# zju3dv/Mirror-NeRF

Measured on AMD Instinct MI355X. Metric: rendered rays/sec (primary+reflected), higher is better.
Workload: dtype f32 carried as hi/lo f16 pairs (f16 MFMA, f32 accumulate; max |diff| to the fp32 chain 3e-6)

## Files before the change

include/mnrf.h:

```cpp
#ifndef MNRF_H
#define MNRF_H

#include <stdint.h>

#ifdef __cplusplus
extern "C" {
#endif

#define MNRF_OK 0
#define MNRF_ERR_ARG (-1)
#define MNRF_ERR_LAUNCH (-2)
#define MNRF_ERR_UNSUPPORTED (-3)

#define MNRF_N_PARAMS 32

#define MNRF_SIGMA_ONLY 1u
#define MNRF_GRAD_NORMAL 2u
#define MNRF_SPLIT_F16 4u

#define MNRF_TCNN_GRAD_F16 16u
#define MNRF_TCNN_GRAD_FIXED 512u
#define MNRF_TCNN_F16 256u
#define MNRF_TCNN_TABLE_F16 1024u
#define MNRF_TCNN_VALU 8u
// ... 114 lines not shown
                         const float* normal, const float* save_invj, const uint64_t* save_mask,
                         float* workspace, float* const* d_params, float* d_xyz, unsigned flags , void* stream);

int mnrf_tcnn_encode(const float* table, const int64_t* offsets17_host, double log2_per_level_scale, int base_resolution,
                     float bound, int64_t B, const float* xyz, int64_t xyz_stride, const float* rays, const float* z_vals,
                     int spr, float* planes, void* stream);

int mnrf_tcnn_encode_flags(const float* table, const int64_t* offsets17_host, double log2_per_level_scale, int base_resolution,
                           float bound, int64_t B, const float* xyz, int64_t xyz_stride, const float* rays, const float* z_vals,
                           int spr, float* planes, unsigned flags, void* stream);
int mnrf_tcnn_table_half(const float* table, int64_t entries, void* table_half, void* stream);

int mnrf_bench_gather(const void* table, int64_t table_bytes, int bytes_per_gather, int64_t n_threads, int iters, float* out,
                      void* stream);

int mnrf_fused_samples_per_ray(void);
int mnrf_field_composite_fused(float* packed, int64_t n_rays, const float* rays, const float* z_vals,
                               const float* dir_emb, int64_t dir_stride, int white_back,
                               float* weights, float* opacity, float* rgb_map, float* depth, float* mirror_mask,
                               float* surf_normal, float* x_surface, void* stream);

#define MNRF_TRAIN_PLANES 256u
#define MNRF_PLANES_Y_HALF 0x100000u
int64_t mnrf_train_planes_bytes(int64_t B);
int64_t mnrf_train_dy_planes_bytes(int64_t B);

int mnrf_field_backward_planes(float* packed, int64_t B, const float* xyz, int64_t xyz_stride,
                               const float* rays, const float* z_vals, int spr,
                               const float* g_sigma, const float* g_rgb, const float* g_pred_normal,
                               const float* g_is_mirror, const float* rgb, const float* pred_normal,
                               const float* is_mirror, const uint64_t* save_mask, const float* save_inv,
                               void* dy_planes, uint32_t* seedmax, float* d_xyz, float* d_dir, const float* keep_mirror,
                               unsigned flags ,
// ... 194 lines not shown
```

mirror_nerf_amd/_lib.py:

```python
import ctypes
import os
import subprocess

import torch

_HERE = os.path.dirname(os.path.abspath(__file__))
LIB_PATH = os.environ.get("MNRF_LIB", os.path.join(_HERE, "libmnrf_hip.so"))
CSRC = os.path.join(_HERE, "csrc")

_c_f = ctypes.c_void_p
_c_i = ctypes.c_void_p
_i64 = ctypes.c_int64
_int = ctypes.c_int
_u32 = ctypes.c_uint
_flt = ctypes.c_float
_str = ctypes.c_void_p

MNRF_SIGMA_ONLY = 1
MNRF_GRAD_NORMAL = 2
MNRF_SPLIT_F16 = 4
MNRF_TCNN_VALU = 8
MNRF_TCNN_F16 = 256
MNRF_TCNN_GRAD_FIXED = 512
MNRF_TCNN_TABLE_F16 = 1024
MNRF_CUT_NORMAL_HEAD = 32
MNRF_CUT_MIRROR_HEAD = 64
MNRF_DW_ACCUMULATE = 128
MNRF_TRAIN_PLANES = 256
MNRF_PLANES_Y_HALF = 0x100000
MNRF_TCNN_GRAD_F16 = 16
MNRF_DETACH_W_MASK = 1
MNRF_DETACH_W_NORMAL = 2
N_PARAMS = 32

SIGNATURES = {
# ... 166 lines not shown
```

mirror_nerf_amd/csrc/mnrf_composite.inc:

```
struct CompMaps {
    float* weights;
    float* opacity; float* rgb_map; float* depth; float* mirror_mask;
    float* surf_normal; float* surf_normal_grad; float* normal_dif; float* x_surface;
    const float* rays;
    int white_back;
};

template <class Src>
__device__ __forceinline__ void composite_ray(const Src& src, int S, int lane, long long ray, const CompMaps& A) {
    float carry = 1.f;
    float a_op = 0.f, a_d = 0.f, a_m = 0.f, a_nd = 0.f;
    float a_c[3] = {0.f, 0.f, 0.f}, a_n[3] = {0.f, 0.f, 0.f}, a_g[3] = {0.f, 0.f, 0.f};
    for (int base = 0; base < S; base += 64) {
        const int s = base + lane;
        const bool in = s < S;
        float alpha = 0.f, zv = 0.f;
        if (in) {
            zv = src.z(s);
            const float delta = s + 1 < S ? src.z(s + 1) - zv : 1e10f;
            float sv = src.sigma(s);
            if (src.has_noise()) sv = sv + src.noise(s);
            alpha = 1.f - expf(-delta * fmaxf(sv, 0.f));
        }
        const float t = in ? (1.f - alpha) + 1e-10f : 1.f;
// ... 18 lines not shown
#pragma unroll
                for (int k = 0; k < 3; ++k) { pn[k] = src.pn(s, k); a_n[k] += pn[k] * w; }
            }
            if (src.has_gn()) {
#pragma unroll
                for (int k = 0; k < 3; ++k) { gn[k] = src.gn(s, k); a_g[k] += gn[k] * w; }
            }
            if (src.has_pn() && src.has_gn()) {
                const float d0 = gn[0] - pn[0], d1 = gn[1] - pn[1], d2 = gn[2] - pn[2];
                a_nd += w * (d0 * d0 + d1 * d1 + d2 * d2);
            }
        }
    }
    a_op = wave_sum(a_op);
    a_d = wave_sum(a_d);
    a_m = wave_sum(a_m);
    a_nd = wave_sum(a_nd);
#pragma unroll
    for (int k = 0; k < 3; ++k) { a_c[k] = wave_sum(a_c[k]); a_n[k] = wave_sum(a_n[k]); a_g[k] = wave_sum(a_g[k]); }
    if (lane == 0) {
        if (A.opacity) A.opacity[ray] = a_op;
        if (A.rgb_map) {
#pragma unroll
            for (int k = 0; k < 3; ++k) A.rgb_map[ray * 3 + k] = A.white_back ? a_c[k] + (1.f - a_op) : a_c[k];
        }
        if (A.depth) A.depth[ray] = a_d;
        if (A.mirror_mask) A.mirror_mask[ray] = a_m;
        if (A.surf_normal) { for (int k = 0; k < 3; ++k) A.surf_normal[ray * 3 + k] = a_n[k]; }
        if (A.surf_normal_grad) { for (int k = 0; k < 3; ++k) A.surf_normal_grad[ray * 3 + k] = a_g[k]; }
        if (A.normal_dif) A.normal_dif[ray] = a_nd;
        if (A.x_surface) {
            const float* r = A.rays + ray * 8;
            for (int k = 0; k < 3; ++k) A.x_surface[ray * 3 + k] = r[k] + r[3 + k] * a_d;
        }
// ... 3 lines not shown
```

mirror_nerf_amd/csrc/mnrf_field.hip:

```cpp
#include <hip/hip_runtime.h>
#include <stdint.h>
#include <stdlib.h>

#include "mnrf_layout.h"
#include "mnrf_field_args.h"

namespace mnrf {

extern __shared__ __attribute__((aligned(16))) char smem[];

namespace s2 {
constexpr int S = 2;
constexpr int MIN_WAVES_PER_SIMD = 1;
constexpr int CHUNK_TILES = 16;
#include "mnrf_field_impl.inc"
#include "mnrf_field_bwd.inc"
}
namespace s1 {
constexpr int S = 1;
constexpr int MIN_WAVES_PER_SIMD = 2;
constexpr int CHUNK_TILES = 16;
#include "mnrf_field_impl.inc"
}

// ... 144 lines not shown
    if (!xyz && B % spr != 0) return mnrf_fail(MNRF_ERR_ARG, "mnrf_field_forward: B not a multiple of spr");
    if (!sigma_only && !dir_emb) return mnrf_fail(MNRF_ERR_ARG, "mnrf_field_forward: dir_emb required unless SIGMA_ONLY");
    if (grad && !normal) return mnrf_fail(MNRF_ERR_ARG, "mnrf_field_forward: GRAD_NORMAL needs the normal output");
    FieldArgs A{packed, flags, (long long)B, xyz, (long long)xyz_stride, rays, z_vals, spr, dir_emb,
                (long long)dir_stride, sigma, rgb, pred_normal, is_mirror, normal, geo_feat};
    const int rc = (flags & MNRF_SPLIT_F16) ? launch_split(A, sigma_only, grad, (hipStream_t)stream)
                 : grad ? s1::launch(A, sigma_only, grad, (hipStream_t)stream)
                        : s2::launch(A, sigma_only, grad, (hipStream_t)stream);
    if (rc != 0) return mnrf_fail(MNRF_ERR_ARG, "mnrf_field_forward: too many samples for one launch");
    return mnrf_check_launch("mnrf_field_forward");
}

extern "C" int mnrf_fused_samples_per_ray(void) { return split48_ray_samples(); }

extern "C" int mnrf_field_composite_fused(float* packed, int64_t n_rays, const float* rays, const float* z_vals,
                                          const float* dir_emb, int64_t dir_stride, int white_back,
                                          float* weights, float* opacity, float* rgb_map, float* depth, float* mirror_mask,
                                          float* surf_normal, float* x_surface, void* stream) {
    if (!packed || !rays || !z_vals || !dir_emb) return mnrf_fail(MNRF_ERR_ARG, "mnrf_field_composite_fused: null pointer");
    if (n_rays < 0) return mnrf_fail(MNRF_ERR_ARG, "mnrf_field_composite_fused: negative ray count");
    if (n_rays == 0) return MNRF_OK;
    if (!split48_enabled())
        return mnrf_fail(MNRF_ERR_UNSUPPORTED, "mnrf_field_composite_fused: needs the 48-samples-per-wave tuning (MNRF_SPLIT48 != 0)");
    const int spr = split48_ray_samples();
    FieldArgs A{packed, MNRF_SPLIT_F16, (long long)n_rays * spr, nullptr, 3, rays, z_vals, spr, dir_emb, (long long)dir_stride,
                nullptr, nullptr, nullptr, nullptr, nullptr, nullptr};
    A.fuse = 1;
    A.white_back = white_back;
    A.f_weights = weights; A.f_opacity = opacity; A.f_rgb_map = rgb_map; A.f_depth = depth; A.f_mirror_mask = mirror_mask;
    A.f_surf_normal = surf_normal; A.f_x_surface = x_surface;
    if (launch_split48(A, false, (hipStream_t)stream) != 0)
        return mnrf_fail(MNRF_ERR_ARG, "mnrf_field_composite_fused: too many samples for one launch");
    return mnrf_check_launch("mnrf_field_composite_fused");
}

static inline int64_t train_tiles(int64_t B) { return (B + s2::WG_SAMPLES - 1) / s2::WG_SAMPLES; }

extern "C" int64_t mnrf_train_save_floats(int64_t B) { return (int64_t)SAVE_FLOATS * B; }
extern "C" int64_t mnrf_train_mask_words(int64_t B) { return train_tiles(B) * N_MASKS * s2::S * s2::WG_THREADS; }
extern "C" int64_t mnrf_train_workspace_floats(int64_t B) { return (int64_t)DY_FLOATS * B + dw_workspace_floats(B); }

static int field_forward_train_impl(float* packed, int64_t B, const float* xyz, int64_t xyz_stride,
                                    const float* rays, const float* z_vals, int spr, const float* dir_emb,
// ... 246 lines not shown
```

mirror_nerf_amd/csrc/mnrf_field_split.hip:

```cpp
#include <hip/hip_runtime.h>
#include <stdint.h>
#include <type_traits>
#include <stdlib.h>

#include "mnrf_layout.h"
#include "mnrf_field_args.h"

namespace mnrf {

extern __shared__ __attribute__((aligned(16))) char smem[];

namespace h2 {
constexpr int S = 2;
constexpr int MIN_WAVES_PER_SIMD = 1;
constexpr int CHUNK_PAIRS = 8;
constexpr int RING_SLOTS = 4;
#include "mnrf_field_split.inc"
}
namespace h2x {
constexpr int S = 2;
constexpr int MIN_WAVES_PER_SIMD = 1;
constexpr int CHUNK_PAIRS = 16;
constexpr int RING_SLOTS = 3;
#include "mnrf_field_split.inc"
// ... 108 lines not shown
        } else if (b >= BIAS_DIR && b < BIAS_DIR + 128) {
            const float* wd = I.wdir[blockIdx.y] + (b - BIAS_DIR) * (W + ENC_DIR);
            double a = 0.0;
            for (int k = 0; k < W; ++k) a = fma((double)wd[k], (double)bias[BIAS_FIN + k], a);
            v = (float)(a + (double)bias[b]);
        }
        packed[OFF_FOLD_BIAS + b] = v;
        return;
    }
    const int pair = (int)(q >> 6);
    const int lane = (int)(q & 63);
    const int row = lane & 15;
    typedef _Float16 h8v __attribute__((ext_vector_type(8)));
    h8v hi, lo;
    for (int j = 0; j < 8; ++j) hi[j] = lo[j] = (_Float16)0.f;
    const int sp = pair < 968 ? pair : (pair < 1036 ? pair + (1036 - 968) : (pair >= 1100 && pair < 1112 ? pair + (1296 - 1100) : -1));
    if (sp >= 0) {
        const char* src = (const char*)(packed + OFF_SPLIT_FWD) + (long long)sp * PAIR_BYTES + lane * 16;
        hi = *(const h8v*)src;
        lo = *(const h8v*)(src + PAIR_BYTES / 2);
    }
    const bool fold_nrm = pair >= 960 && pair < 968 && row >= 1 && row <= 3;
    const bool fold_dir = pair >= 1036 && pair < 1100;
    if (fold_nrm || fold_dir) {
        const int T = fold_nrm ? pair - 960 : (pair - 1036) / 8;
        const int c0 = 32 * T + 4 * (lane >> 4);
        const float* a = fold_nrm ? I.wn2[blockIdx.y] + (row - 1) * 128 : I.wdir[blockIdx.y] + (16 * ((pair - 1036) % 8) + row) * (W + ENC_DIR);
        const float* bm = fold_nrm ? I.wn1[blockIdx.y] : I.wfin[blockIdx.y];
        const int K = fold_nrm ? 128 : W;
        double acc[8];
        for (int j = 0; j < 8; ++j) acc[j] = 0.0;
        for (int k = 0; k < K; ++k) {
            const double ak = (double)a[k];
            const float* bk = bm + (long long)k * W + c0;
#pragma unroll
            for (int c = 0; c < 4; ++c) {
                acc[c] = fma(ak, (double)bk[c], acc[c]);
                acc[4 + c] = fma(ak, (double)bk[16 + c], acc[4 + c]);
            }
        }
        bool bad = false;
#pragma unroll
// ... 28 lines not shown
```

mirror_nerf_amd/csrc/mnrf_field_split.inc:

```
constexpr int CHUNK_BYTES = CHUNK_PAIRS * PAIR_BYTES;
constexpr int WAVES = 4;
constexpr int WG_THREADS = 64 * WAVES;
constexpr int WG_SAMPLES = WAVES * S * 16;
constexpr int PIECES = CHUNK_BYTES / TILE_BYTES / WAVES;
constexpr int U = 2;
constexpr int PF = S == 3 ? 2 : 4;
constexpr int NBUF = PF + U;
typedef unsigned u32x4 __attribute__((ext_vector_type(4)));
typedef unsigned u32x2 __attribute__((ext_vector_type(2)));
typedef _Float16 h2v __attribute__((ext_vector_type(2)));
struct StoreCtx {
    __amdgpu_buffer_rsrc_t rsrc;
    __amdgpu_buffer_rsrc_t rsrc_lo;
    char* base;
    int lane;
    int soff;
    h2v fac[S];
};
__device__ __forceinline__ __amdgpu_buffer_rsrc_t plane_rsrc(char* sample_block) {
    return __builtin_amdgcn_make_buffer_rsrc(sample_block, 0, 0x7fffffff, 0x00020000);
}
static_assert(CHUNK_PAIRS / U == PIECES, "one LDS-DMA piece per wave per unit");
constexpr int LDS_RING = RING_SLOTS * CHUNK_BYTES;
constexpr int LDS_BIAS = LDS_RING;
// ... 21 lines not shown
struct CompLdsSrc {
    const float* f;
    bool pn_on, mir_on;
    __device__ __forceinline__ bool has_noise() const { return false; }
    __device__ __forceinline__ bool has_rgb() const { return true; }
    __device__ __forceinline__ bool has_mirror() const { return mir_on; }
    __device__ __forceinline__ bool has_pn() const { return pn_on; }
    __device__ __forceinline__ bool has_gn() const { return false; }
    __device__ __forceinline__ float z(int s) const { return f[8 * WG_SAMPLES + s]; }
    __device__ __forceinline__ float sigma(int s) const { return f[s]; }
    __device__ __forceinline__ float noise(int) const { return 0.f; }
    __device__ __forceinline__ float rgb(int s, int k) const { return f[(1 + k) * WG_SAMPLES + s]; }
    __device__ __forceinline__ float mirror(int s) const { return f[7 * WG_SAMPLES + s]; }
    __device__ __forceinline__ float pn(int s, int k) const { return f[(4 + k) * WG_SAMPLES + s]; }
    __device__ __forceinline__ float gn(int, int) const { return 0.f; }
};

__device__ __forceinline__ unsigned long long enc_out_of_range(const float (&x)[S][3]) {
    bool big = false;
#pragma unroll
    for (int s = 0; s < S; ++s) big |= !(fabsf(x[s][0]) < ENC_RANGE_LIMIT && fabsf(x[s][1]) < ENC_RANGE_LIMIT && fabsf(x[s][2]) < ENC_RANGE_LIMIT);
    return __builtin_amdgcn_ballot_w64(big);
}

template <int N>
__device__ __forceinline__ void split_b(const float (&x)[S][N], u32x4 (&hi)[S][N / 8], u32x4 (&lo)[S][N / 8],
                                        unsigned long long& sat, float limit = F16_MAX) {
    float tmax = 0.f;
#pragma unroll
    for (int s = 0; s < S; ++s)
// ... 337 lines not shown
            sat_track<ACT == 1>(tmax, v[2], v[3]);
            hi[s][nb >> 1][2 * (nb & 1)] = h0;
            hi[s][nb >> 1][2 * (nb & 1) + 1] = h1;
            lo[s][nb >> 1][2 * (nb & 1)] = l0;
            lo[s][nb >> 1][2 * (nb & 1) + 1] = l1;
        }
        if (WANT_MASK) ((uint64_t*)(smem + LDS_MASK))[(layer * S + s) * WG_THREADS + tid] = m;
    }
    sat_flush(sat, tmax);
}

__device__ __forceinline__ float sigmoidf_(float x) { return 1.f / (1.f + expf(-x)); }



template <bool SIGMA_ONLY, bool GRAD, bool PLANES = false, bool FUSE = false>
__global__ __launch_bounds__(WG_THREADS, MIN_WAVES_PER_SIMD) void field_split_kernel(FieldArgs A) {
    static_assert(!PLANES || (GRAD && !SIGMA_ONLY && S == 2), "operand planes: the training forward (32 samples per wave)");
    static_assert(!FUSE || (S == 3 && !SIGMA_ONLY && !GRAD), "ray-fused compositing: the 192-sample fine pass");
    constexpr bool FOLD = !SIGMA_ONLY && !GRAD;
    float* const fz = (float*)(smem + LDS_FUSE);
    constexpr bool PERSIST = S == 3;
    if constexpr (PLANES) {
        if (A.n_live) {
            long long bl = (long long)*A.n_live * A.spr;
            bl = bl < 0 ? 0 : bl;
            if (bl < A.B) A.B = bl;
        }
        if ((long long)blockIdx.x * WG_SAMPLES >= A.B) return;
    }
    const bool queued = PERSIST && A.tile_queue != nullptr;
    const int wave = __builtin_amdgcn_readfirstlane(threadIdx.x >> 6);
    int tile = blockIdx.x;
    int round = 0;
// ... 268 lines not shown
    };
    {
        f32x4 acc[S][1];
        init_bias<1>(acc, BIAS_SIG, gq());
        gemm_part<8, 1, 960, HP>(acc, hh, hl, st, wave, lane16);
        if (FUSE) {
            if (gq() == 0) {
#pragma unroll
                for (int s = 0; s < S; ++s) fz[wave * (S * 16) + s * 16 + m15()] = acc[s][0][0];
            }
        } else if (A.sigma && g == 0) {
#pragma unroll
            for (int s = 0; s < S; ++s)
                if (sval(s)) out_store(A.sigma + sidx(s), acc[s][0][0]);
        }
        if constexpr (FOLD) put_normal(acc, std::integral_constant<int, 1>{});
    }

    if (!SIGMA_ONLY) {
        if constexpr (!FOLD) {
            u32x4 nh[S][4], nl[S][4];
            {
                f32x4 acc[S][8];
                init_bias<8>(acc, BIAS_NRM1, gq());
                gemm_part<8, 8, 968, HP, ST0>(acc, hh, hl, st, wave, lane16, at_h(7, 0));
                if (keep) save_acc<8, 0>(A.save_x + (long long)SEC_HN * A.B, 128, 0, acc, idx, valid, g, unused_bits);
                acc_to_b<8, 0, false>(nh, nl, acc, 0, tid, st.sat);
                if constexpr (S == 2) { if (pl) store_planes<4, 4>(sc, SEC_HN / 16, nh, nl); }
            }
            f32x4 acc[S][1];
            init_bias<1>(acc, BIAS_NRM2, gq());
            gemm_part<4, 1, 1032>(acc, nh, nl, st, wave, lane16);
            put_normal(acc, std::integral_constant<int, 0>{});
        }
        {
            u32x4 mh[S][4], ml[S][4];
            {
                f32x4 acc[S][8];
                init_bias<8>(acc, BIAS_MIR1, gq());
                gemm_part<8, 8, FOLD ? 968 : 1036, HP, ST4>(acc, hh, hl, st, wave, lane16, at_h(7, 4));
                if (keep) {
                    uint64_t bits[S];
                    save_acc<8, 2>(A.save_x + (long long)SEC_HM * A.B, 128, 0, acc, idx, valid, g, bits);
#pragma unroll
                    for (int s = 0; s < S; ++s) gmask[(9 * S + s) * WG_THREADS + tid] = bits[s];
                } else if (GRAD && pl) {
                    store_sign_mask<8>(acc, gmask + (9 * S) * WG_THREADS + tid);
                }
                acc_to_b<8, 2, false>(mh, ml, acc, 0, tid, st.sat);
                if constexpr (S == 2) { if (pl) store_planes<4, 4>(sc, SEC_HM / 16, mh, ml); }
            }
            f32x4 acc[S][1];
            init_bias<1>(acc, BIAS_MIR2, gq());
            gemm_part<4, 1, FOLD ? 1032 : 1100>(acc, mh, ml, st, wave, lane16);
            if (FUSE) {
                if (gq() == 0) {
#pragma unroll
                    for (int s = 0; s < S; ++s) fz[7 * WG_SAMPLES + wave * (S * 16) + s * 16 + m15()] = sigmoidf_(acc[s][0][0]);
                }
            } else if (A.is_mirror && g == 0) {
#pragma unroll
                for (int s = 0; s < S; ++s)
                    if (sval(s)) out_store(A.is_mirror + sidx(s), sigmoidf_(acc[s][0][0]));
            }
        }
        const auto view_operands = [&](u32x4 (&vh)[S][1], u32x4 (&vl)[S][1]) {
            float de[S][8];
            const int gv = gq();
            const int spr = opaque_spr();
#pragma unroll
            for (int s = 0; s < S; ++s) {
                const float* dp = A.dir_emb + (long long)(sidx(s) / spr) * A.dir_stride;
#pragma unroll
                for (int t = 0; t < 8; ++t) {
                    const int e = 16 * (t >> 2) + 4 * gv + (t & 3);
                    de[s][t] = e < ENC_DIR ? dp[e] : 0.f;
                }
            }
            if (keep) save_bform<8>(A.save_x + (long long)SEC_DIRE * A.B, 32, de, idx, valid, g);
            split_b<8>(de, vh, vl, st.sat);
            if constexpr (S == 2) { if (pl) store_planes<1, 1>(sc, SEC_DIRE / 16, vh, vl); }
        };
        {
            u32x4 dh[S][4], dl[S][4];
            if constexpr (FOLD) {
                u32x4 vh[S][1], vl[S][1];
                view_operands(vh, vl);
                f32x4 acc[S][8];
                init_bias<8>(acc, BIAS_DIR, gq());
                gemm_part<8, 8, 1036, HP>(acc, hh, hl, st, wave, lane16);
                gemm_part<1, 8, 1100>(acc, vh, vl, st, wave, lane16);
                acc_to_b<8, 1, false>(dh, dl, acc, 0, tid, st.sat);
            } else {
                u32x4 fh[S][8], fl[S][8];
                {
                    f32x4 acc[S][16];
                    init_bias<16>(acc, BIAS_FIN, gq());
                    gemm_part<8, 16, 1104, HP>(acc, hh, hl, st, wave, lane16);
                    if (keep) save_acc<16, 0>(A.save_x + (long long)SEC_FIN * A.B, 256, 0, acc, idx, valid, g, unused_bits);
                    acc_to_b<16, 0, false>(fh, fl, acc, 0, tid, st.sat);
                    if constexpr (S == 2) { if (pl) store_planes<8, 8>(sc, SEC_FIN / 16, fh, fl); }
                }
                u32x4 vh[S][1], vl[S][1];
                view_operands(vh, vl);
                f32x4 acc[S][8];
                init_bias<8>(acc, BIAS_DIR, gq());
                gemm_part<8, 8, 1232>(acc, fh, fl, st, wave, lane16);
                gemm_part<1, 8, 1296>(acc, vh, vl, st, wave, lane16);
                if (keep) {
                    uint64_t bits[S];
                    save_acc<8, 1>(A.save_x + (long long)SEC_HD * A.B, 128, 0, acc, idx, valid, g, bits);
#pragma unroll
                    for (int s = 0; s < S; ++s) gmask[(8 * S + s) * WG_THREADS + tid] = bits[s];
                } else if (GRAD && pl) {
                    store_sign_mask<8>(acc, gmask + (8 * S) * WG_THREADS + tid);
                }
                acc_to_b<8, 1, false>(dh, dl, acc, 0, tid, st.sat);
                if constexpr (S == 2) { if (pl) store_planes<4, 4>(sc, SEC_HD / 16, dh, dl); }
            }
            f32x4 acc[S][1];
            init_bias<1>(acc, BIAS_RGB, gq());
            gemm_part<4, 1, FOLD ? 1108 : 1304>(acc, dh, dl, st, wave, lane16);
            if (FUSE) {
                if (gq() == 0) {
#pragma unroll
                    for (int s = 0; s < S; ++s) {
                        const int q = wave * (S * 16) + s * 16 + (int)m15();
                        fz[1 * WG_SAMPLES + q] = sigmoidf_(acc[s][0][0]);
                        fz[2 * WG_SAMPLES + q] = sigmoidf_(acc[s][0][1]);
                        fz[3 * WG_SAMPLES + q] = sigmoidf_(acc[s][0][2]);
                    }
                }
            } else if (A.rgb && g == 0) {
#pragma unroll
                for (int s = 0; s < S; ++s)
                    if (sval(s)) {
                        float* o = A.rgb + (long long)sidx(s) * 3;
                        out_store(o, sigmoidf_(acc[s][0][0]));
                        out_store(o + 1, sigmoidf_(acc[s][0][1]));
                        out_store(o + 2, sigmoidf_(acc[s][0][2]));
                    }
            }
        }
    }

    if (GRAD) {
        open_stream<false>(st, A.packed + OFF_SPLIT_BWD, wave, lane);
        prime_stream(st, lane16);
        float gr[S][64];
        {
            const f32x4* ws = (const f32x4*)(smem + LDS_BIAS) + (BIAS_WSIG >> 2);
#pragma unroll
            for (int nb = 0; nb < 16; ++nb) {
                const f32x4 v = ws[nb * 4 + g];
#pragma unroll
                for (int s = 0; s < S; ++s)
#pragma unroll
                    for (int r = 0; r < 4; ++r) gr[s][4 * nb + r] = v[r];
// ... 70 lines not shown
                const float n0 = -d0, n1 = -d1, n2 = -d2;
                const float sq = n0 * n0 + n1 * n1 + n2 * n2;
                const float inv = 1.f / sqrtf(fmaxf(sq, 1.1920928955078125e-07f));
                float* o = A.normal + (long long)idx[s] * 3;
                o[0] = n0 * inv; o[1] = n1 * inv; o[2] = n2 * inv;
                if (A.save_invj) A.save_invj[idx[s]] = sq > 1.1920928955078125e-07f ? inv : -inv;
            }
        }
    }
    sat_all |= st.sat;
    enc_all |= enc_range;
    if (FUSE) {
        __syncthreads();
        if (wave == 0) {
            const long long ray = tile;
            const CompLdsSrc src{fz, A.f_surf_normal != nullptr, A.f_mirror_mask != nullptr};
            const CompMaps out{A.f_weights ? A.f_weights + ray * WG_SAMPLES : nullptr, A.f_opacity, A.f_rgb_map, A.f_depth, A.f_mirror_mask,
                               A.f_surf_normal, nullptr, nullptr, A.f_x_surface, A.rays, A.white_back};
            int cl;
            asm volatile("v_mbcnt_lo_u32_b32 %0, -1, 0\n\tv_mbcnt_hi_u32_b32 %0, -1, %0" : "=v"(cl));
            composite_ray(src, WG_SAMPLES, cl, ray, out);
        }
    }
    if (!queued) break;
    close_stream();
    __syncthreads();
    tile = __builtin_amdgcn_readfirstlane(((volatile int*)(smem + LDS_TILEQ))[round & 1]);
    ++round;
    if (tile >= A.n_tiles) break;
    }
    guard_report(A.packed, sat_all, enc_all, MNRF_GUARD_IN_FORWARD);
    close_stream();
    int last_lane;
    asm volatile("v_mbcnt_lo_u32_b32 %0, -1, 0\n\tv_mbcnt_hi_u32_b32 %0, -1, %0" : "=v"(last_lane));
    if (queued && wave == 0 && last_lane == 0) {
        if (atomicAdd(A.tile_queue + 1, 1) == (int)gridDim.x - 1) {
            atomicExch(A.tile_queue, 0);
            atomicExch(A.tile_queue + 1, 0);
        }
    }
}

inline int launch(const FieldArgs& A, bool sigma_only, bool grad, hipStream_t s) {
    const long long blocks64 = (A.B + WG_SAMPLES - 1) / WG_SAMPLES;
    if (blocks64 > 0x7fffffff || A.B > 0x7fffffffLL) return -1;
    dim3 grid((unsigned)blocks64);
    const dim3 block(WG_THREADS);
    if (S == 3 && A.tile_queue) {
        if (A.n_tiles != (int)blocks64 || A.resident < 1 || A.resident > A.n_tiles) return -1;
        grid = dim3((unsigned)A.resident);
    }
    if (sigma_only && !grad) hipLaunchKernelGGL((field_split_kernel<true, false>), grid, block, LDS_BYTES, s, A);
    else if (!sigma_only && !grad && S == 3 && A.fuse)
        hipLaunchKernelGGL((field_split_kernel<false, false, false, S == 3>), grid, block, LDS_BYTES_FUSE, s, A);
    else if (!sigma_only && !grad) hipLaunchKernelGGL((field_split_kernel<false, false>), grid, block, LDS_BYTES, s, A);
#ifndef MNRF_SPLIT_NO_GRAD
    else if (sigma_only && grad) hipLaunchKernelGGL((field_split_kernel<true, true>), grid, block, LDS_BYTES_GRAD, s, A);
    else if (S == 2 && A.save_planes) hipLaunchKernelGGL((field_split_kernel<false, true, S == 2>), grid, block, LDS_BYTES_GRAD, s, A);
    else hipLaunchKernelGGL((field_split_kernel<false, true>), grid, block, LDS_BYTES_GRAD, s, A);
#else
    else return -1;
#endif
    return 0;
}
```

mirror_nerf_amd/csrc/mnrf_field_split3.hip:

```cpp
#include <hip/hip_runtime.h>
#include <stdint.h>
#include <type_traits>
#include <stdlib.h>

#include "mnrf_layout.h"
#include "mnrf_field_args.h"

namespace mnrf {

extern __shared__ __attribute__((aligned(16))) char smem[];

namespace h3 {
constexpr int S = 3;
constexpr int MIN_WAVES_PER_SIMD = 1;
constexpr int CHUNK_PAIRS = 8;
constexpr int RING_SLOTS = 4;
#define MNRF_SPLIT_NO_GRAD
#include "mnrf_field_split.inc"
#undef MNRF_SPLIT_NO_GRAD
}

bool split48_enabled() {
    static const bool v = [] { const char* e = getenv("MNRF_SPLIT48"); return !(e && atoi(e) == 0); }();
    return v;
// ... 20 lines not shown
    A.resident = resident;
    return true;
}

int launch_split48(const FieldArgs& A0, bool sigma_only, hipStream_t s) {
    FieldArgs A = A0;
    A.tile_queue = nullptr;
    if (tile_queue_slot(A)) {
        if (hipMemsetAsync(A.tile_queue, 0, 2 * sizeof(int), s) != hipSuccess) A.tile_queue = nullptr;
    }
    static const bool once = [] {
        (void)hipFuncSetAttribute((const void*)h3::field_split_kernel<true, false>, hipFuncAttributeMaxDynamicSharedMemorySize, h3::LDS_BYTES);
        (void)hipFuncSetAttribute((const void*)h3::field_split_kernel<false, false>, hipFuncAttributeMaxDynamicSharedMemorySize, h3::LDS_BYTES);
        (void)hipFuncSetAttribute((const void*)h3::field_split_kernel<false, false, false, true>, hipFuncAttributeMaxDynamicSharedMemorySize,
                                   h3::LDS_BYTES_FUSE);
        return true;
    }();
    (void)once;
    return h3::launch(A, sigma_only, false, s);
}

int split48_ray_samples() { return h3::WG_SAMPLES; }

}
```

mirror_nerf_amd/csrc/mnrf_layout.h:

```cpp
#pragma once
#include <stdint.h>

namespace mnrf {

constexpr int W = 256;
constexpr int ENC_XYZ = 63;
constexpr int ENC_DIR = 27;
constexpr int NFREQ_XYZ = 10;
constexpr int NFREQ_DIR = 4;

constexpr int TILE_FLOATS = 256;
constexpr int TILE_BYTES = 1024;
constexpr int PAD_TILES = 16;

enum PartKind : int {
    KIND_H = 0,
    KIND_ENC = 1,
    KIND_DIR = 2,
};

__host__ __device__ inline int enc_col(int t, int g) {
    const int P = 8 * g + (t >> 1);
    const int s = t & 1;
    if (P < 30) return 3 + 6 * (P / 3) + 3 * s + (P % 3);
// ... 42 lines not shown
constexpr int64_t PACKED_F32_FLOATS = OFF_HBWD + (int64_t)HBWD_TILES * TILE_FLOATS;

constexpr int PAIR_BYTES = 2048;
constexpr int SPLIT_END_PAD = 16;
__host__ __device__ constexpr int padded_pairs(int n) { return (n + SPLIT_END_PAD - 1) / SPLIT_END_PAD * SPLIT_END_PAD; }
constexpr int SPLIT_FWD_USED_SIGMA = 960 + 8;
constexpr int SPLIT_FWD_USED = SPLIT_FWD_USED_SIGMA + 64 + 4 + 64 + 4 + 128 + 64 + 8 + 4;
constexpr int SPLIT_FWD_PAIRS = padded_pairs(SPLIT_FWD_USED);
constexpr int SPLIT_BWD_PAIRS = 3 * 128 + 32 + 128 + 3 * 128 + 32;
constexpr int SPLIT_HBWD_PAIRS = padded_pairs(8 + 64 + 8 + 128 + 8 + 64 + 8 + 64);
constexpr int64_t OFF_SPLIT_FWD = PACKED_F32_FLOATS;
constexpr int64_t OFF_SPLIT_BWD = OFF_SPLIT_FWD + (int64_t)SPLIT_FWD_PAIRS * (PAIR_BYTES / 4);
constexpr int64_t OFF_SPLIT_HBWD = OFF_SPLIT_BWD + (int64_t)SPLIT_BWD_PAIRS * (PAIR_BYTES / 4);
constexpr int64_t SPLIT_TAIL_FLOATS = 2 * 16 * (PAIR_BYTES / 4);
constexpr int FOLD_REGION_PAIRS = 1328;
constexpr int SPLIT_FOLD_USED = 960 + 8 + 64 + 4 + 64 + 8 + 4;
constexpr int SPLIT_FOLD_PAIRS = padded_pairs(SPLIT_FOLD_USED);
constexpr int64_t OFF_FOLD_FWD = OFF_SPLIT_HBWD + (int64_t)SPLIT_HBWD_PAIRS * (PAIR_BYTES / 4);
constexpr int64_t OFF_FOLD_BIAS = OFF_FOLD_FWD + (int64_t)SPLIT_FOLD_PAIRS * (PAIR_BYTES / 4) + SPLIT_TAIL_FLOATS;
constexpr int64_t PACKED_FLOATS = OFF_FOLD_FWD + (int64_t)FOLD_REGION_PAIRS * (PAIR_BYTES / 4) + SPLIT_TAIL_FLOATS;
constexpr int TQ_PAIRS = 8;
constexpr int64_t OFF_TILE_QUEUE = PACKED_FLOATS - 1 - 2 * TQ_PAIRS;
constexpr int64_t OFF_REDUCE_PAIR = OFF_TILE_QUEUE - 2;
constexpr int DEVICE_STATE_WORDS = 2 + 2 * TQ_PAIRS + 1;
static_assert(OFF_FOLD_BIAS + BIAS_FLOATS <= OFF_REDUCE_PAIR, "the folded stream, its read-ahead tail and its bias block fit the reserved region");

constexpr int SEC_ENC = 0;
constexpr int SEC_H = 64;
constexpr int SEC_FIN = 2112;
constexpr int SEC_DIRE = 2368;
constexpr int SEC_HD = 2400;
constexpr int SEC_HN = 2528;
// ... 69 lines not shown
```

mirror_nerf_amd/recursion.py:

```python
import ctypes
import os
from collections import defaultdict
from types import SimpleNamespace

import torch
from torch import nn

from . import _lib
from .mirror_nerf import Embedding, MirrorNeRF
from .rendering import render_rays

RAY_FORWARD_OFFSET = 0.1
JITTER_RAYS = 262144

PLACE_MIRROR_PRESETS = {
    "plane_x": (
        ("livingroom", dict(position=0.0, normal=(-1.0, 0.0, 0.0), rect=(-1.0, 1.0, -0.5, 0.5))),
        ("washroom", dict(position=-1.0, normal=(1.0, 0.0, 0.0), rect=(-1.0, 1.0, -1.0, 0.75))),
        ("office", dict(position=1.0, normal=(1.0, 0.0, 0.0), rect=(-1.0, 1.0, -1.0, 0.75))),
        (None, dict(position=-1.0, normal=(1.0, 0.0, 0.0), rect=(-1.0, 1.0, -0.5, 0.5))),
    ),
    "plane_y": (
        ("washroom", dict(position=1.3, normal=(0.0, -1.0, 0.0), rect=(-1.0, 1.0, -1.0, 1.0))),
        ("livingroom", dict(position=1.65, normal=(0.0, -1.0, 0.0), rect=(-0.3, 1.5, -0.5, 1.0))),
# ... 422 lines not shown
        noise_iter = iter(noise_iter)
    to_cpu = kwargs.get("to_cpu", True)
    maps_only = bool(kwargs.get("maps_only", to_cpu == "maps"))
    rough = getattr(args, "app_control_mirror_roughness", False)
    batch_jitter = kwargs.get("batch_jitter", noise_iter is None)
    one_field = getattr(args, "only_one_field", False)
    fine_epoch = getattr(args, "only_one_field_fine_epoch", 2)
    sel = "fine" if (N_importance > 0 and not one_field) else "coarse"

    def draw(n, dev):
        if noise_iter is not None:
            return next(noise_iter).to(dev).float().contiguous()
        return torch.randn(n, 3, device=dev)

    def stage_a(rays_chunk, level, host_flags=None, slot=0):
        r = render_rays(models, embeddings, rays_chunk, N_samples, use_disp, 0, 0, N_importance, chunk,
                        white_back, test_time=test_time,
                        compute_normal=trace_flag and (not args.predict_normal),
                        only_one_field=one_field, only_one_field_fine_epoch=fine_epoch,
                        current_epoch=fine_epoch + 1, _guard=False, _maps_only=maps_only)
        r[f"rgb_{sel}_reflect"] = torch.zeros_like(r[f"rgb_{sel}"])
        r[f"depth_{sel}_reflect"] = torch.zeros_like(r[f"depth_{sel}"])
        mask = None
        for key in (f"mirror_mask_{sel}", "mirror_mask_fine", "mirror_mask_coarse"):
            if key in r:
                mask = r[key]
                break
        last = level >= args.max_recursive_level or not (trace_flag or place)
        edit = None
        if place and not last:
            edit = lambda flag: _place_mirror(r, rays_chunk, sel, plane, args.near, flag)
        pending, any_mirror = None, False
        if mask is not None:
            if host_flags is not None and not last and rays_chunk.shape[0]:
                pending = _threshold_async(mask, host_flags, slot, edit)
# ... 15 lines not shown
        if level >= args.max_recursive_level:
            trace = False
        if not trace or N == 0:
            return r
        mask = (mask != 0).float()
        normal = _pick_normal(r, sel)
        nn0 = draw(N, dev) if rough else None
        sec, index, rdir = _reflect(rays_chunk, r[f"x_surface_{sel}"], normal, mask, only_in, nn0, noise_std)
        r["reflect_direction"] = rdir
        if sec.shape[0] > 0:
            if subst:
                _transform_rays(sec, xform)
                r2 = render_rays(system_sub.models, system_sub.embeddings, sec.contiguous(), N_samples, use_disp, 0, 0,
                                 N_importance, chunk, white_back, test_time=test_time, compute_normal=False,
                                 only_one_field=one_field, only_one_field_fine_epoch=fine_epoch,
                                 current_epoch=fine_epoch + 1, _guard=False, _maps_only=True)
            else:
                r2 = recurse(sec.contiguous(), level + 1)
            if rough:
                times = args.trace_ray_times
                if batch_jitter and times > 0:
                    mj = max(1, r2[f"rgb_{sel}"].shape[0])
                    g = 0
                    while g < times:
                        n_g = max(1, min(times - g, JITTER_RAYS // mj))
                        secs = [_reflect(rays_chunk, r[f"x_surface_{sel}"], normal, mask, True, draw(N, dev), noise_std,
                                         want_dir=False)[0] for _ in range(n_g)]
                        r3 = recurse(torch.cat(secs, 0).contiguous(), level + 1)
                        for typ in ("coarse", "fine"):
                            if f"rgb_{typ}" in r2:
                                for piece in r3[f"rgb_{typ}"].view(n_g, -1, 3).unbind(0):
# ... 76 lines not shown
```

mirror_nerf_amd/rendering.py:

```python
import torch

from . import _lib
from .autograd import CompositeFn, EmbedFn, FieldFn
from .mirror_nerf import field_forward
from .weights import params_of

__all__ = ["render_rays", "sample_pdf"]

_LINSPACE = {}


def _linspace01(n, device):
    key = (n, str(device))
    t = _LINSPACE.get(key)
    if t is None:
        t = torch.linspace(0, 1, n).to(device)
        _LINSPACE[key] = t
    return t


def _n_freqs(emb):
    n = getattr(emb, "N_freqs", None)
    if n is None:
        raise RuntimeError("embeddings must expose N_freqs (Embedding modules)")
# ... 115 lines not shown
        per_pass = {"_noise_coarse": (r_fc, r_cc, de_c), "_noise_fine": (r_ff, r_cf, de_f)}
    else:
        z_vals = f(N, N_samples)
        if N:
            _lib.check(L.mnrf_sample_coarse_n(p(rays), N, p(z_steps), N_samples, int(bool(use_disp)), float(perturb),
                                              p(prand), p(z_vals), p(n_live), _lib.stream()), "mnrf_sample_coarse")

    has_fine = "fine" in models
    results = {}

    def inference_fused(model, typ, z):
        from . import mirror_nerf as _mn
        from .weights import folded_of
        if _mn.precision_of(model) != "split" or z.shape[1] != L.mnrf_fused_samples_per_ray():
            return False
        has_m, has_n = getattr(model, "predict_mirror_mask", True), getattr(model, "predict_normal", True)
        opacity, rgb_map, depth, xs = f(N), f(N, 3), f(N), f(N, 3)
        mask = f(N) if has_m else None
        sn = f(N, 3) if has_n else None
        if _mn.LAUNCH_LOG is not None:
            e0, e1 = torch.cuda.Event(enable_timing=True), torch.cuda.Event(enable_timing=True)
            e0.record()
        rc = L.mnrf_field_composite_fused(p(folded_of(model)), N, p(rays), p(z), p(dir_emb), dir_emb.shape[1], int(bool(white_back)),
                                          None, p(opacity), p(rgb_map), p(depth), p(mask), p(sn), p(xs), _lib.stream())
        if rc == -3:
            return False
        _lib.check(rc, "mnrf_field_composite_fused")
        if _mn.LAUNCH_LOG is not None:
            e1.record()
            _mn.LAUNCH_LOG.append((_lib.MNRF_SPLIT_F16 | 0x2000, N * z.shape[1], e0, e1))
        results[f"opacity_{typ}"] = opacity
        results[f"z_vals_{typ}"] = z
        results[f"rgb_{typ}"] = rgb_map
        results[f"depth_{typ}"] = depth
        if has_m:
            results[f"mirror_mask_{typ}"] = mask
        if has_n:
            results[f"surface_normal_{typ}"] = sn
        results[f"_x_surface_{typ}"] = xs
        return True

    def inference(model, typ, z, noise_key):
        S = z.shape[1]
        sigma_only = typ == "coarse" and test_time and has_fine
        B = N * S
        if train and not sigma_only and N:
            return inference_train(model, typ, z, noise_key)
        if (kwargs.get("_maps_only") and test_time and not sigma_only and N and not hashgrid and not compute_normal
                and noise_std == 0 and kwargs.get(noise_key) is None and inference_fused(model, typ, z)):
            return
        if N and hashgrid:
            o = model.field(B, rays=rays, z_vals=z, spr=S, dirs=dir_emb, sigma_only=sigma_only,
                            grad_normal=compute_normal and not sigma_only)
        elif N:
# ... 131 lines not shown
            if kwargs.get("_z_fine") is not None:
                return kwargs["_z_fine"].float().contiguous()
            if "_z_fine_fused" in results:
                return results.pop("_z_fine_fused")
            return sample_pdf(z_vals, results["weights_coarse"].detach(), N_importance, det=(perturb == 0), u=given_u(), n_live=n_live)

        if kwargs.get("only_one_field", False):
            if kwargs.get("current_epoch", 0) > kwargs.get("only_one_field_fine_epoch", 2):
                inference(models["coarse"], "coarse", fine_depths(), "_noise_fine")
        else:
            inference(models["fine"], "fine", fine_depths(), "_noise_fine")

    results.pop("_z_fine_fused", None)
    for typ in ("coarse", "fine"):
        xs = results.pop(f"_x_surface_{typ}", None)
        if f"depth_{typ}" in results:
            results[f"x_surface_{typ}"] = xs
    if kwargs.get("_guard", True) and N and not hashgrid:
        from .mirror_nerf import check_guard, release_transient
        if check_guard(list(models.values())):
            try:
                return render_rays(models, embeddings, rays, N_samples, use_disp, perturb, noise_std, N_importance, chunk,
                                   white_back, test_time, **kwargs)
            finally:
                release_transient(list(models.values()))
    return results
```

Measured before the change: 1.826 million.

## Add rgb/depth-only fused fine pass skipping mirror and normal heads for reflected rays

Adds a flag to the fused field+composite kernel that builds a variant without the mirror-mask head, the folded normal output or the x_surface output. The recursion path uses it for secondary rays and for the deepest recursion level, where only colour and depth are consumed. The folded weight stream is reordered so the mirror-head weights come after the direction/RGB parts, which lets the mirror head be dropped at the tail. Wave reductions in compositing are also skipped for channels the source lacks. The cost is an extra kernel instantiation, and any caller that expected mirror or normal outputs at those levels no longer receives them.

After: 1.875 million, median of 6. 1.03x the previous value.

```diff
diff --git a/include/mnrf.h b/include/mnrf.h
--- a/include/mnrf.h
+++ b/include/mnrf.h
@@ -152,9 +152,11 @@
 int mnrf_bench_gather(const void* table, int64_t table_bytes, int bytes_per_gather, int64_t n_threads, int iters, float* out,
                       void* stream);
 
+#define MNRF_FUSED_WHITE_BACK 1u
+#define MNRF_FUSED_RGB_DEPTH 2u
 int mnrf_fused_samples_per_ray(void);
 int mnrf_field_composite_fused(float* packed, int64_t n_rays, const float* rays, const float* z_vals,
-                               const float* dir_emb, int64_t dir_stride, int white_back,
+                               const float* dir_emb, int64_t dir_stride, int flags,
                                float* weights, float* opacity, float* rgb_map, float* depth, float* mirror_mask,
                                float* surf_normal, float* x_surface, void* stream);
 
diff --git a/mirror_nerf_amd/_lib.py b/mirror_nerf_amd/_lib.py
--- a/mirror_nerf_amd/_lib.py
+++ b/mirror_nerf_amd/_lib.py
@@ -19,6 +19,8 @@
 MNRF_SIGMA_ONLY = 1
 MNRF_GRAD_NORMAL = 2
 MNRF_SPLIT_F16 = 4
+MNRF_FUSED_WHITE_BACK = 1
+MNRF_FUSED_RGB_DEPTH = 2
 MNRF_TCNN_VALU = 8
 MNRF_TCNN_F16 = 256
 MNRF_TCNN_GRAD_FIXED = 512
diff --git a/mirror_nerf_amd/csrc/mnrf_composite.inc b/mirror_nerf_amd/csrc/mnrf_composite.inc
--- a/mirror_nerf_amd/csrc/mnrf_composite.inc
+++ b/mirror_nerf_amd/csrc/mnrf_composite.inc
@@ -56,10 +56,14 @@
     }
     a_op = wave_sum(a_op);
     a_d = wave_sum(a_d);
-    a_m = wave_sum(a_m);
-    a_nd = wave_sum(a_nd);
+    if (src.has_mirror()) a_m = wave_sum(a_m);
+    if (src.has_pn() && src.has_gn()) a_nd = wave_sum(a_nd);
 #pragma unroll
-    for (int k = 0; k < 3; ++k) { a_c[k] = wave_sum(a_c[k]); a_n[k] = wave_sum(a_n[k]); a_g[k] = wave_sum(a_g[k]); }
+    for (int k = 0; k < 3; ++k) {
+        if (src.has_rgb()) a_c[k] = wave_sum(a_c[k]);
+        if (src.has_pn()) a_n[k] = wave_sum(a_n[k]);
+        if (src.has_gn()) a_g[k] = wave_sum(a_g[k]);
+    }
     if (lane == 0) {
         if (A.opacity) A.opacity[ray] = a_op;
         if (A.rgb_map) {
diff --git a/mirror_nerf_amd/csrc/mnrf_field.hip b/mirror_nerf_amd/csrc/mnrf_field.hip
--- a/mirror_nerf_amd/csrc/mnrf_field.hip
+++ b/mirror_nerf_amd/csrc/mnrf_field.hip
@@ -182,19 +182,23 @@
 extern "C" int mnrf_fused_samples_per_ray(void) { return split48_ray_samples(); }
 
 extern "C" int mnrf_field_composite_fused(float* packed, int64_t n_rays, const float* rays, const float* z_vals,
-                                          const float* dir_emb, int64_t dir_stride, int white_back,
+                                          const float* dir_emb, int64_t dir_stride, int flags,
                                           float* weights, float* opacity, float* rgb_map, float* depth, float* mirror_mask,
                                           float* surf_normal, float* x_surface, void* stream) {
     if (!packed || !rays || !z_vals || !dir_emb) return mnrf_fail(MNRF_ERR_ARG, "mnrf_field_composite_fused: null pointer");
     if (n_rays < 0) return mnrf_fail(MNRF_ERR_ARG, "mnrf_field_composite_fused: negative ray count");
+    if (flags & ~(int)(MNRF_FUSED_WHITE_BACK | MNRF_FUSED_RGB_DEPTH)) return mnrf_fail(MNRF_ERR_ARG, "mnrf_field_composite_fused: unknown flag bits");
+    const bool rgb_depth = flags & MNRF_FUSED_RGB_DEPTH;
+    if (rgb_depth && (mirror_mask || surf_normal))
+        return mnrf_fail(MNRF_ERR_ARG, "mnrf_field_composite_fused: MNRF_FUSED_RGB_DEPTH evaluates neither the mirror head nor the normal map");
     if (n_rays == 0) return MNRF_OK;
     if (!split48_enabled())
         return mnrf_fail(MNRF_ERR_UNSUPPORTED, "mnrf_field_composite_fused: needs the 48-samples-per-wave tuning (MNRF_SPLIT48 != 0)");
     const int spr = split48_ray_samples();
     FieldArgs A{packed, MNRF_SPLIT_F16, (long long)n_rays * spr, nullptr, 3, rays, z_vals, spr, dir_emb, (long long)dir_stride,
                 nullptr, nullptr, nullptr, nullptr, nullptr, nullptr};
-    A.fuse = 1;
-    A.white_back = white_back;
+    A.fuse = rgb_depth ? 2 : 1;
+    A.white_back = (flags & MNRF_FUSED_WHITE_BACK) != 0;
     A.f_weights = weights; A.f_opacity = opacity; A.f_rgb_map = rgb_map; A.f_depth = depth; A.f_mirror_mask = mirror_mask;
     A.f_surf_normal = surf_normal; A.f_x_surface = x_surface;
     if (launch_split48(A, false, (hipStream_t)stream) != 0)
diff --git a/mirror_nerf_amd/csrc/mnrf_field_split.hip b/mirror_nerf_amd/csrc/mnrf_field_split.hip
--- a/mirror_nerf_amd/csrc/mnrf_field_split.hip
+++ b/mirror_nerf_amd/csrc/mnrf_field_split.hip
@@ -146,18 +146,21 @@
     typedef _Float16 h8v __attribute__((ext_vector_type(8)));
     h8v hi, lo;
     for (int j = 0; j < 8; ++j) hi[j] = lo[j] = (_Float16)0.f;
-    const int sp = pair < 968 ? pair : (pair < 1036 ? pair + (1036 - 968) : (pair >= 1100 && pair < 1112 ? pair + (1296 - 1100) : -1));
+    const int sp = pair < FOLD_POS_DIR ? pair
+                 : pair < FOLD_POS_VIEW ? -1
+                 : pair < FOLD_POS_MIR1 ? pair + (1296 - FOLD_POS_VIEW)
+                 : pair < SPLIT_FOLD_USED ? pair + (1036 - FOLD_POS_MIR1) : -1;
     if (sp >= 0) {
         const char* src = (const char*)(packed + OFF_SPLIT_FWD) + (long long)sp * PAIR_BYTES + lane * 16;
         hi = *(const h8v*)src;
         lo = *(const h8v*)(src + PAIR_BYTES / 2);
     }
     const bool fold_nrm = pair >= 960 && pair < 968 && row >= 1 && row <= 3;
-    const bool fold_dir = pair >= 1036 && pair < 1100;
+    const bool fold_dir = pair >= FOLD_POS_DIR && pair < FOLD_POS_VIEW;
     if (fold_nrm || fold_dir) {
-        const int T = fold_nrm ? pair - 960 : (pair - 1036) / 8;
+        const int T = fold_nrm ? pair - 960 : (pair - FOLD_POS_DIR) / 8;
         const int c0 = 32 * T + 4 * (lane >> 4);
-        const float* a = fold_nrm ? I.wn2[blockIdx.y] + (row - 1) * 128 : I.wdir[blockIdx.y] + (16 * ((pair - 1036) % 8) + row) * (W + ENC_DIR);
+        const float* a = fold_nrm ? I.wn2[blockIdx.y] + (row - 1) * 128 : I.wdir[blockIdx.y] + (16 * ((pair - FOLD_POS_DIR) % 8) + row) * (W + ENC_DIR);
         const float* bm = fold_nrm ? I.wn1[blockIdx.y] : I.wfin[blockIdx.y];
         const int K = fold_nrm ? 128 : W;
         double acc[8];
diff --git a/mirror_nerf_amd/csrc/mnrf_field_split.inc b/mirror_nerf_amd/csrc/mnrf_field_split.inc
--- a/mirror_nerf_amd/csrc/mnrf_field_split.inc
+++ b/mirror_nerf_amd/csrc/mnrf_field_split.inc
@@ -59,6 +59,10 @@
     __device__ __forceinline__ float mirror(int s) const { return f[7 * WG_SAMPLES + s]; }
     __device__ __forceinline__ float pn(int s, int k) const { return f[(4 + k) * WG_SAMPLES + s]; }
     __device__ __forceinline__ float gn(int, int) const { return 0.f; }
+};
+struct CompLdsSrcRgbDepth : CompLdsSrc {
+    __device__ __forceinline__ bool has_mirror() const { return false; }
+    __device__ __forceinline__ bool has_pn() const { return false; }
 };
 
 __device__ __forceinline__ unsigned long long enc_out_of_range(const float (&x)[S][3]) {
@@ -426,10 +430,11 @@
 
 
 
-template <bool SIGMA_ONLY, bool GRAD, bool PLANES = false, bool FUSE = false>
-__global__ __launch_bounds__(WG_THREADS, MIN_WAVES_PER_SIMD) void field_split_kernel(FieldArgs A) {
+template <bool SIGMA_ONLY, bool GRAD, bool PLANES, bool FUSE, bool RGB_DEPTH>
+__device__ __forceinline__ void field_split_body(FieldArgs A) {
     static_assert(!PLANES || (GRAD && !SIGMA_ONLY && S == 2), "operand planes: the training forward (32 samples per wave)");
     static_assert(!FUSE || (S == 3 && !SIGMA_ONLY && !GRAD), "ray-fused compositing: the 192-sample fine pass");
+    static_assert(!RGB_DEPTH || FUSE, "rgb / depth only: a variant of the ray-fused pass");
     constexpr bool FOLD = !SIGMA_ONLY && !GRAD;
     float* const fz = (float*)(smem + LDS_FUSE);
     constexpr bool PERSIST = S == 3;
@@ -728,7 +733,7 @@
             for (int s = 0; s < S; ++s)
                 if (sval(s)) out_store(A.sigma + sidx(s), acc[s][0][0]);
         }
-        if constexpr (FOLD) put_normal(acc, std::integral_constant<int, 1>{});
+        if constexpr (FOLD && !RGB_DEPTH) put_normal(acc, std::integral_constant<int, 1>{});
     }
 
     if (!SIGMA_ONLY) {
@@ -747,12 +752,12 @@
             gemm_part<4, 1, 1032>(acc, nh, nl, st, wave, lane16);
             put_normal(acc, std::integral_constant<int, 0>{});
         }
-        {
+        const auto mirror_head = [&]() {
             u32x4 mh[S][4], ml[S][4];
             {
                 f32x4 acc[S][8];
                 init_bias<8>(acc, BIAS_MIR1, gq());
-                gemm_part<8, 8, FOLD ? 968 : 1036, HP, ST4>(acc, hh, hl, st, wave, lane16, at_h(7, 4));
+                gemm_part<8, 8, FOLD ? FOLD_POS_MIR1 : 1036, HP, ST4>(acc, hh, hl, st, wave, lane16, at_h(7, 4));
                 if (keep) {
                     uint64_t bits[S];
                     save_acc<8, 2>(A.save_x + (long long)SEC_HM * A.B, 128, 0, acc, idx, valid, g, bits);
@@ -766,7 +771,7 @@
             }
             f32x4 acc[S][1];
             init_bias<1>(acc, BIAS_MIR2, gq());
-            gemm_part<4, 1, FOLD ? 1032 : 1100>(acc, mh, ml, st, wave, lane16);
+            gemm_part<4, 1, FOLD ? FOLD_POS_MIR2 : 1100>(acc, mh, ml, st, wave, lane16);
             if (FUSE) {
                 if (gq() == 0) {
 #pragma unroll
@@ -777,7 +782,8 @@
                 for (int s = 0; s < S; ++s)
                     if (sval(s)) out_store(A.is_mirror + sidx(s), sigmoidf_(acc[s][0][0]));
             }
-        }
+        };
+        if constexpr (!FOLD) mirror_head();
         const auto view_operands = [&](u32x4 (&vh)[S][1], u32x4 (&vl)[S][1]) {
             float de[S][8];
             const int gv = gq();
@@ -802,8 +808,8 @@
                 view_operands(vh, vl);
                 f32x4 acc[S][8];
                 init_bias<8>(acc, BIAS_DIR, gq());
-                gemm_part<8, 8, 1036, HP>(acc, hh, hl, st, wave, lane16);
-                gemm_part<1, 8, 1100>(acc, vh, vl, st, wave, lane16);
+                gemm_part<8, 8, FOLD_POS_DIR, HP>(acc, hh, hl, st, wave, lane16);
+                gemm_part<1, 8, FOLD_POS_VIEW>(acc, vh, vl, st, wave, lane16);
                 acc_to_b<8, 1, false>(dh, dl, acc, 0, tid, st.sat);
             } else {
                 u32x4 fh[S][8], fl[S][8];
@@ -834,7 +840,7 @@
             }
             f32x4 acc[S][1];
             init_bias<1>(acc, BIAS_RGB, gq());
-            gemm_part<4, 1, FOLD ? 1108 : 1304>(acc, dh, dl, st, wave, lane16);
+            gemm_part<4, 1, FOLD ? FOLD_POS_RGB : 1304>(acc, dh, dl, st, wave, lane16);
             if (FUSE) {
                 if (gq() == 0) {
 #pragma unroll
@@ -856,6 +862,7 @@
                     }
             }
         }
+        if constexpr (FOLD && !RGB_DEPTH) mirror_head();
     }
 
     if (GRAD) {
@@ -956,12 +963,18 @@
         __syncthreads();
         if (wave == 0) {
             const long long ray = tile;
-            const CompLdsSrc src{fz, A.f_surf_normal != nullptr, A.f_mirror_mask != nullptr};
-            const CompMaps out{A.f_weights ? A.f_weights + ray * WG_SAMPLES : nullptr, A.f_opacity, A.f_rgb_map, A.f_depth, A.f_mirror_mask,
-                               A.f_surf_normal, nullptr, nullptr, A.f_x_surface, A.rays, A.white_back};
             int cl;
             asm volatile("v_mbcnt_lo_u32_b32 %0, -1, 0\n\tv_mbcnt_hi_u32_b32 %0, -1, %0" : "=v"(cl));
-            composite_ray(src, WG_SAMPLES, cl, ray, out);
+            if constexpr (RGB_DEPTH) {
+                const CompMaps out{A.f_weights ? A.f_weights + ray * WG_SAMPLES : nullptr, A.f_opacity, A.f_rgb_map, A.f_depth, nullptr,
+                                   nullptr, nullptr, nullptr, A.f_x_surface, A.rays, A.white_back};
+                composite_ray(CompLdsSrcRgbDepth{fz, false, false}, WG_SAMPLES, cl, ray, out);
+            } else {
+                const CompLdsSrc src{fz, A.f_surf_normal != nullptr, A.f_mirror_mask != nullptr};
+                const CompMaps out{A.f_weights ? A.f_weights + ray * WG_SAMPLES : nullptr, A.f_opacity, A.f_rgb_map, A.f_depth, A.f_mirror_mask,
+                                   A.f_surf_normal, nullptr, nullptr, A.f_x_surface, A.rays, A.white_back};
+                composite_ray(src, WG_SAMPLES, cl, ray, out);
+            }
         }
     }
     if (!queued) break;
@@ -983,6 +996,16 @@
     }
 }
 
+template <bool SIGMA_ONLY, bool GRAD, bool PLANES = false, bool FUSE = false>
+__global__ __launch_bounds__(WG_THREADS, MIN_WAVES_PER_SIMD) void field_split_kernel(FieldArgs A) {
+    field_split_body<SIGMA_ONLY, GRAD, PLANES, FUSE, false>(A);
+}
+template <bool ON = true>
+__global__ __launch_bounds__(WG_THREADS, MIN_WAVES_PER_SIMD) void field_split_kernel_rgb_depth(FieldArgs A) {
+    field_split_body<false, false, false, ON, ON>(A);
+}
+
+template <bool UNUSED = false>
 inline int launch(const FieldArgs& A, bool sigma_only, bool grad, hipStream_t s) {
     const long long blocks64 = (A.B + WG_SAMPLES - 1) / WG_SAMPLES;
     if (blocks64 > 0x7fffffff || A.B > 0x7fffffffLL) return -1;
@@ -993,7 +1016,9 @@
         grid = dim3((unsigned)A.resident);
     }
     if (sigma_only && !grad) hipLaunchKernelGGL((field_split_kernel<true, false>), grid, block, LDS_BYTES, s, A);
-    else if (!sigma_only && !grad && S == 3 && A.fuse)
+    else if (!sigma_only && !grad && S == 3 && A.fuse == 2) {
+        if constexpr (S == 3) hipLaunchKernelGGL((field_split_kernel_rgb_depth<>), grid, block, LDS_BYTES_FUSE, s, A);
+    } else if (!sigma_only && !grad && S == 3 && A.fuse)
         hipLaunchKernelGGL((field_split_kernel<false, false, false, S == 3>), grid, block, LDS_BYTES_FUSE, s, A);
     else if (!sigma_only && !grad) hipLaunchKernelGGL((field_split_kernel<false, false>), grid, block, LDS_BYTES, s, A);
 #ifndef MNRF_SPLIT_NO_GRAD
diff --git a/mirror_nerf_amd/csrc/mnrf_field_split3.hip b/mirror_nerf_amd/csrc/mnrf_field_split3.hip
--- a/mirror_nerf_amd/csrc/mnrf_field_split3.hip
+++ b/mirror_nerf_amd/csrc/mnrf_field_split3.hip
@@ -58,6 +58,7 @@
         (void)hipFuncSetAttribute((const void*)h3::field_split_kernel<false, false>, hipFuncAttributeMaxDynamicSharedMemorySize, h3::LDS_BYTES);
         (void)hipFuncSetAttribute((const void*)h3::field_split_kernel<false, false, false, true>, hipFuncAttributeMaxDynamicSharedMemorySize,
                                    h3::LDS_BYTES_FUSE);
+        (void)hipFuncSetAttribute((const void*)h3::field_split_kernel_rgb_depth<>, hipFuncAttributeMaxDynamicSharedMemorySize, h3::LDS_BYTES_FUSE);
         return true;
     }();
     (void)once;
diff --git a/mirror_nerf_amd/csrc/mnrf_layout.h b/mirror_nerf_amd/csrc/mnrf_layout.h
--- a/mirror_nerf_amd/csrc/mnrf_layout.h
+++ b/mirror_nerf_amd/csrc/mnrf_layout.h
@@ -80,8 +80,14 @@
 constexpr int64_t OFF_SPLIT_HBWD = OFF_SPLIT_BWD + (int64_t)SPLIT_BWD_PAIRS * (PAIR_BYTES / 4);
 constexpr int64_t SPLIT_TAIL_FLOATS = 2 * 16 * (PAIR_BYTES / 4);
 constexpr int FOLD_REGION_PAIRS = 1328;
-constexpr int SPLIT_FOLD_USED = 960 + 8 + 64 + 4 + 64 + 8 + 4;
+constexpr int FOLD_POS_DIR = 960 + 8;
+constexpr int FOLD_POS_VIEW = FOLD_POS_DIR + 64;
+constexpr int FOLD_POS_RGB = FOLD_POS_VIEW + 8;
+constexpr int FOLD_POS_MIR1 = FOLD_POS_RGB + 4;
+constexpr int FOLD_POS_MIR2 = FOLD_POS_MIR1 + 64;
+constexpr int SPLIT_FOLD_USED = FOLD_POS_MIR2 + 4;
 constexpr int SPLIT_FOLD_PAIRS = padded_pairs(SPLIT_FOLD_USED);
+static_assert(SPLIT_FOLD_USED == 960 + 8 + 64 + 4 + 64 + 8 + 4, "the folded stream holds every folded part once");
 constexpr int64_t OFF_FOLD_FWD = OFF_SPLIT_HBWD + (int64_t)SPLIT_HBWD_PAIRS * (PAIR_BYTES / 4);
 constexpr int64_t OFF_FOLD_BIAS = OFF_FOLD_FWD + (int64_t)SPLIT_FOLD_PAIRS * (PAIR_BYTES / 4) + SPLIT_TAIL_FLOATS;
 constexpr int64_t PACKED_FLOATS = OFF_FOLD_FWD + (int64_t)FOLD_REGION_PAIRS * (PAIR_BYTES / 4) + SPLIT_TAIL_FLOATS;
diff --git a/mirror_nerf_amd/recursion.py b/mirror_nerf_amd/recursion.py
--- a/mirror_nerf_amd/recursion.py
+++ b/mirror_nerf_amd/recursion.py
@@ -460,11 +460,13 @@
         return torch.randn(n, 3, device=dev)
 
     def stage_a(rays_chunk, level, host_flags=None, slot=0):
+        rgb_depth = 1 <= level == args.max_recursive_level and not rough
         r = render_rays(models, embeddings, rays_chunk, N_samples, use_disp, 0, 0, N_importance, chunk,
                         white_back, test_time=test_time,
                         compute_normal=trace_flag and (not args.predict_normal),
                         only_one_field=one_field, only_one_field_fine_epoch=fine_epoch,
-                        current_epoch=fine_epoch + 1, _guard=False, _maps_only=maps_only)
+                        current_epoch=fine_epoch + 1, _guard=False, _maps_only=maps_only or rgb_depth,
+                        _rgb_depth_only=rgb_depth)
         r[f"rgb_{sel}_reflect"] = torch.zeros_like(r[f"rgb_{sel}"])
         r[f"depth_{sel}_reflect"] = torch.zeros_like(r[f"depth_{sel}"])
         mask = None
@@ -510,7 +512,7 @@
                 r2 = render_rays(system_sub.models, system_sub.embeddings, sec.contiguous(), N_samples, use_disp, 0, 0,
                                  N_importance, chunk, white_back, test_time=test_time, compute_normal=False,
                                  only_one_field=one_field, only_one_field_fine_epoch=fine_epoch,
-                                 current_epoch=fine_epoch + 1, _guard=False, _maps_only=True)
+                                 current_epoch=fine_epoch + 1, _guard=False, _maps_only=True, _rgb_depth_only=True)
             else:
                 r2 = recurse(sec.contiguous(), level + 1)
             if rough:
diff --git a/mirror_nerf_amd/rendering.py b/mirror_nerf_amd/rendering.py
--- a/mirror_nerf_amd/rendering.py
+++ b/mirror_nerf_amd/rendering.py
@@ -153,21 +153,25 @@
         from .weights import folded_of
         if _mn.precision_of(model) != "split" or z.shape[1] != L.mnrf_fused_samples_per_ray():
             return False
-        has_m, has_n = getattr(model, "predict_mirror_mask", True), getattr(model, "predict_normal", True)
-        opacity, rgb_map, depth, xs = f(N), f(N, 3), f(N), f(N, 3)
+        rgb_depth = bool(kwargs.get("_rgb_depth_only"))
+        has_m = not rgb_depth and getattr(model, "predict_mirror_mask", True)
+        has_n = not rgb_depth and getattr(model, "predict_normal", True)
+        opacity, rgb_map, depth = f(N), f(N, 3), f(N)
+        xs = None if rgb_depth else f(N, 3)
         mask = f(N) if has_m else None
         sn = f(N, 3) if has_n else None
+        flags = (_lib.MNRF_FUSED_WHITE_BACK if white_back else 0) | (_lib.MNRF_FUSED_RGB_DEPTH if rgb_depth else 0)
         if _mn.LAUNCH_LOG is not None:
             e0, e1 = torch.cuda.Event(enable_timing=True), torch.cuda.Event(enable_timing=True)
             e0.record()
-        rc = L.mnrf_field_composite_fused(p(folded_of(model)), N, p(rays), p(z), p(dir_emb), dir_emb.shape[1], int(bool(white_back)),
+        rc = L.mnrf_field_composite_fused(p(folded_of(model)), N, p(rays), p(z), p(dir_emb), dir_emb.shape[1], flags,
                                           None, p(opacity), p(rgb_map), p(depth), p(mask), p(sn), p(xs), _lib.stream())
         if rc == -3:
             return False
         _lib.check(rc, "mnrf_field_composite_fused")
         if _mn.LAUNCH_LOG is not None:
             e1.record()
-            _mn.LAUNCH_LOG.append((_lib.MNRF_SPLIT_F16 | 0x2000, N * z.shape[1], e0, e1))
+            _mn.LAUNCH_LOG.append((_lib.MNRF_SPLIT_F16 | 0x2000 | (0x4000 if rgb_depth else 0), N * z.shape[1], e0, e1))
         results[f"opacity_{typ}"] = opacity
         results[f"z_vals_{typ}"] = z
         results[f"rgb_{typ}"] = rgb_map
@@ -176,7 +180,8 @@
             results[f"mirror_mask_{typ}"] = mask
         if has_n:
             results[f"surface_normal_{typ}"] = sn
-        results[f"_x_surface_{typ}"] = xs
+        if xs is not None:
+            results[f"_x_surface_{typ}"] = xs
         return True
 
     def inference(model, typ, z, noise_key):
@@ -338,7 +343,7 @@
     results.pop("_z_fine_fused", None)
     for typ in ("coarse", "fine"):
         xs = results.pop(f"_x_surface_{typ}", None)
-        if f"depth_{typ}" in results:
+        if xs is not None and f"depth_{typ}" in results:
             results[f"x_surface_{typ}"] = xs
     if kwargs.get("_guard", True) and N and not hashgrid:
         from .mirror_nerf import check_guard, release_transient
```
